# Senpai-sama06/real-time-audio-visual-zooming

Hardware: AMD Instinct MI355X
Metric: beamformed TF-bins/sec (2-ch, 1024-pt STFT) + SIR dB delta vs reference (higher is better)
Workload: dtype f32

## Files before the change

### real-time-audio-visual-zooming_amd/csrc/avz_chain_analysis.hpp

```cpp
#pragma once
#include "avz_chain_common.hpp"
#include "avz_chain_exact.hpp"

namespace avz {
template <int N, int MASK, bool IRM, class TW>
__device__ __forceinline__ void analysis_item(const ChainArgs& A, unsigned char* lds, int c,
                                              int b, int p, int P, int slot, const TW& tw_reg,
                                              const LaneConst<N>& K, int seq) {
  using C = KCfg<N>;
  using G = CGeo<N>;
  constexpr int NT = G::NT, H = G::H, F = G::F, NSLOT = G::NSLOT, BPT = G::BPT, PPL = C::PPL;
  constexpr int FB = (MASK == MASK_IBM) ? NSLOT / 2 : NSLOT;
  static_assert(kChunk % FB == 0, "steps tile the chunk");
  constexpr bool REFBITS = N == 1024 && MASK == MASK_IBM && !IRM && !std::is_same<TW, NoTw>::value;
  constexpr bool SHARE = N == 1024 && MASK != MASK_IPD && !std::is_same<TW, NoTw>::value;
  constexpr bool DLT = MASK == MASK_IBM && !REFBITS;

  const int tid = threadIdx.x;
  const int wave = __builtin_amdgcn_readfirstlane(tid >> 6);
  const int lane = tid & 63;
  const int L = utt_len(A, b);
  const int T = (L + H - 1) / H + 1;
  const int nch = (T + kChunk - 1) / kChunk;
  if (L < N || c >= nch) return;
  if (c == 0 && p == 0 && tid == 0) {
    A.peak_u[b] = 0u;
    if (A.peak && A.normalize != NORM_PEAK) A.peak[b] = 0.0f;
  }
  const int t0 = c * kChunk;
  const int nframes = min(kChunk, T - t0);
  constexpr int SA = kChunk / FB;
  const int s_lo = p * SA / P;
  const int nstep = min((nframes + FB - 1) / FB, (p + 1) * SA / P);
  uint32_t* const pendw = reinterpret_cast<uint32_t*>(lds + G::MISC_OFF + 32 + 12 * (seq & 1));
  if (MASK == MASK_IBM && tid == 0) {
    int z = 0;
    opaque_i(z);
    pendw[0] = (uint32_t)z;
    pendw[1] = (uint32_t)z;
    pendw[2] = (uint32_t)z;
  }

  const typename C::Fft fft = K.fft;
  LaneMap<N> lm;
  {
    int ln = threadIdx.x & 63;
    opaque_i(ln);
    lm.init(ln);
  }
  const float cert_raw = A.ibm_cert * (2.0f / N);
  const WinCoef<N> wc = K.wc;
  const int my_slot = wave * C::FPW + lm.grp;
  cf* my_spec = slot_ptr<N>(lds, my_slot);
  const bool ref = (MASK == MASK_IBM) && (wave * C::FPW >= FB);
  const int my_frame = ref ? my_slot - FB : my_slot;
  const int wave_frame0 = ref ? wave * C::FPW - FB : wave * C::FPW;

  const float* mixb = A.mix + (long long)b * A.mix_stride;
  rsrc_t r_re = make_rsrc(mixb, L), r_im = make_rsrc(mixb + A.ch_stride, L);
  if constexpr (MASK == MASK_IBM) {
    if (ref) {
      r_re = make_rsrc(A.ref_tgt + (long long)b * A.ref_stride, L);
      r_im = make_rsrc(A.ref_int + (long long)b * A.ref_stride, L);
    }
  }
  cf v[PPL];
  auto issue_loads = [&](int step) {
    if constexpr (SHARE) {
      const int sp = (t0 + step * FB + wave_frame0) * H - N / 2 + lm.in0;
      if (t0 + step * FB + wave_frame0 >= 1)
        pair_loads<true>(v, r_re, r_im, sp, lm.grp);
      else
        pair_loads<false>(v, r_re, r_im, sp, lm.grp);
      return;
    }
    const int s0 = (t0 + step * FB + my_frame) * H - N / 2 + lm.in0;
    if (t0 + step * FB + wave_frame0 >= 1) {
// ... 3 lines not shown
      });
    } else {
      static_for<0, PPL>([&](auto r) {
        v[r].x = bload(r_re, s0 + C::IN_STRIDE * r);
        v[r].y = bload(r_im, s0 + C::IN_STRIDE * r);
      });
    }
  };

  constexpr bool IL_LOADS = N == 1024 && !std::is_same<TW, NoTw>::value;
  const rsrc_t r_none = make_rsrc(nullptr, 0);
  rsrc_t rn_re = r_none, rn_im = r_none;
  int sp_next = 0;
  auto load_reg = [&](auto kc) {
    constexpr int k = decltype(kc)::value;
    if constexpr (SHARE) {
      if constexpr (k < 16) {
        const int e = sp_next + 1024 * lm.grp + 32 * k;
        v[k].x = bload_nn(rn_re, e);
        v[k].y = bload_nn(rn_im, e);
      } else if constexpr ((k - 16) % 2 == 0) {
        const int e = sp_next + 512 + 32 * (k - 16) + 32 * lm.grp;
        v[k].x = bload_nn(rn_re, e);
        v[k].y = bload_nn(rn_im, e);
      }
    } else {
      v[k].x = bload_nn(rn_re, sp_next + C::IN_STRIDE * k);
      v[k].y = bload_nn(rn_im, sp_next + C::IN_STRIDE * k);
    }
  };

  Acc32 acc[BPT];
  uint32_t bits[BPT];
  uint32_t dfr[BPT];
  int ipd_clear_n[BPT];
#pragma unroll
  for (int j = 0; j < BPT; ++j) {
    acc[j].zero();
    bits[j] = 0u;
    dfr[j] = 0u;
    ipd_clear_n[j] = 0;
  }
  static_assert(!IRM || MASK == MASK_IBM, "IRM needs the references");
  float* const gain = IRM ? A.pf_gain + ((long long)b * A.nchunk + c) * kChunk * F : nullptr;
  const bool nyq_wave = (wave == G::NWAVE - 1);
  Acc32 an, adc;
  an.zero();
  adc.zero();
  uint32_t nyq_bits = 0u, nyq_dfr = 0u;
  float wone[BPT];
#pragma unroll
  for (int j = 0; j < BPT; ++j) wone[j] = (MASK == MASK_IPD && j == 0 && tid == 0) ? 0.0f : 1.0f;

  AVZ_STAMP_DECL();
  issue_loads(s_lo);
  lds_barrier();
  AVZ_STAMP_INIT();
  for (int step = s_lo; step < nstep; ++step) {
    const int f0 = t0 + step * FB;
    const bool live = f0 + wave_frame0 < T;
#ifdef AVZ_STAMPS
    asm volatile("s_waitcnt vmcnt(0)" ::: "memory");
    AVZ_STAMP(0);
#endif
    if (live) {
      if constexpr (SHARE) pair_finish(v);
      float eg0 = 0.0f, eg1 = eg0;
      if constexpr (REFBITS) {
        if (ref) {
          const float eg = group32_sum(frame_energy(v));
          int e0 = __builtin_amdgcn_readlane(__float_as_int(eg), 0);
          int e1 = __builtin_amdgcn_readlane(__float_as_int(eg), 32);
          const bool o0 = (uint32_t)e0 - A.ibm_en_lo > A.ibm_en_span;
          const bool o1 = (uint32_t)e1 - A.ibm_en_lo > A.ibm_en_span;
          if ((o0 || o1) && A.ibm_cert > 0.0f) {
            uint32_t nz = 0u;
            static_for<0, 32>([&](auto r) { nz |= __float_as_uint(v[r].x) | __float_as_uint(v[r].y); });
            const unsigned long long any = __ballot((nz << 1) != 0u);
            const bool f0 = o0 && (uint32_t)any != 0u, f1 = o1 && (any >> 32) != 0ull;
            if (f0 || f1) {
              const bool mine = lm.grp ? f1 : f0;
              static_for<0, 32>([&](auto r) {
                v[r].x = mine ? 0.0f : v[r].x;
                v[r].y = mine ? 0.0f : v[r].y;
              });
              e0 = f0 ? 0x7f800000 : e0;
              e1 = f1 ? 0x7f800000 : e1;
            }
          }
          eg0 = __int_as_float(e0);
          eg1 = __int_as_float(e1);
        }
      }
      if constexpr (MASK == MASK_IPD) {
        bool same = true;
        static_for<0, PPL>([&](auto r) {
          same &= __float_as_uint(v[r].x) == __float_as_uint(v[r].y);
        });
        const unsigned long long nb = __ballot(!same);
        const bool ident = (C::FPW == 1) ? nb == 0ull : ((nb >> (32 * lm.grp)) & 0xffffffffull) == 0ull;
        if ((lane & (64 / C::FPW - 1)) == 0) lds[G::MISC_OFF + my_slot] = ident ? 1 : 0;
      }
      if constexpr (IL_LOADS) {
        const bool more = step + 1 < nstep;
        rn_re = more ? r_re : r_none;
        rn_im = more ? r_im : r_none;
        sp_next = (t0 + (step + 1) * FB + (SHARE ? wave_frame0 : my_frame)) * H - N / 2 + lm.in0;
      }
      float en = 0.0f;
      if constexpr (!IL_LOADS) {
        window_fft<N>(v, wc, fft, my_spec, lm, NoAfter{}, (DLT && ref) ? &en : nullptr);
      } else if constexpr (REFBITS) {
        uint32_t um = 0u;
        if (step + 1 < nstep) {
          if (ref)
            um = window_fft_reg_ibm_bits(v, wc, fft, my_spec, tw_reg, lm, eg0, eg1, cert_raw, en,
// ... 178 lines not shown
        const bool dc = (j == 0 && tid == 0);
        if (dc) f = 0u;
        ipd_clear_n[j] += dc ? 0 : nvalid - __popc(f);
        while (f) {
          const int i = __builtin_ctz(f);
          f &= f - 1u;
          const cf* Zm = slot_ptr<N>(lds, i);
          cf x0, x1;
          split_pair2(Zm[kb], Zm[kp], x0, x1);
          const float w = ((ident_w >> (8 * i)) & 1ull) ? 0.01f : ipd_weight_exact(x0, x1);
          acc[j].add(x0, x1, w - 1.0f, w);
        }
      }
    }
    if (nyq_wave) {
      bool noise = false, nunc = false;
      if (lane < nvalid) {
        int ln = lane;
        opaque_i(ln);
        const cf* Zm = slot_ptr<N>(lds, ln);
        cf y0, y1, zr{0, 0};
        split_pair2(Zm[N / 2], Zm[N / 2], y0, y1);
        if constexpr (MASK == MASK_IBM) zr = slot_ptr<N>(lds, FB + ln)[N / 2];
        float wn;
        float mn = bin_mask<MASK>(A, b, y0, y1, zr, zr, N / 2, f0 + lane, noise, wn);
        if (MASK == MASK_IPD && ((ident_w >> (8 * lane)) & 1ull)) wn = mn = 0.01f;
        if (MASK == MASK_IBM &&
            ibm_uncertain(zr, zr, reinterpret_cast<const float*>(lds + G::MISC_OFF + 16)[lane])) {
          noise = false;
          wn = mn = 0.0f;
          nunc = true;
          atomicOr(pendw, 1u << (step * FB + lane));
        }
        an.add(y0, y1, wn, mn);
        if constexpr (MASK == MASK_IPD) {
          cf d0, d1;
          const cf z0 = Zm[0];
          split_pair2(z0, z0, d0, d1);
          const float wd = ((ident_w >> (8 * lane)) & 1ull) ? 0.01f : ipd_weight_exact(d0, d1);
          adc.add(d0, d1, wd, wd);
        }
        if constexpr (IRM) gain[(step * FB + lane) * F + N / 2] = irm_gain(zr, zr);
      }
      const unsigned long long bal = __ballot(noise);
      nyq_bits |= ((uint32_t)bal & ((1u << FB) - 1u)) << (step * FB);
      if constexpr (MASK == MASK_IBM)
        nyq_dfr |= ((uint32_t)__ballot(nunc) & ((1u << FB) - 1u)) << (step * FB);
    }
    AVZ_STAMP(12);
    lds_barrier();
    AVZ_STAMP(2);
  }

  if constexpr (MASK == MASK_IBM) {
    const uint32_t pend = pendw[0], full = pendw[1];
    const uint32_t big = REFBITS ? pendw[2] : pend;
    KArgs& Ak = kernarg_chain_args();
    const int gxi = (Ak.max_frames + kChunk - 1) / kChunk;
    const int unit = slot < 0 ? b * gxi + c : gxi * Ak.batch + slot;
    if (nyq_wave && lane == 0) {
      reinterpret_cast<uint4*>(Ak.xpend)[unit] = make_uint4(pend, full, nyq_dfr, big);
      if (pend) *reinterpret_cast<uint32_t*>(lds + G::MISC_OFF + 56) |= 1u << min(seq, 31);
    }
    if (DLT && pend != 0u) {
#pragma unroll
      for (int j = 0; j < BPT; ++j) Ak.xdfr[(long long)unit * F + tid + j * NT] = dfr[j];
    }
  }

  float* Pt = slot < 0 ? A.part + ((long long)b * A.nchunk + c) * 5 * F
                       : A.tpart + (long long)slot * 5 * F;
  uint32_t* MW = A.mwords + ((long long)b * A.nchunk + c) * F;
  const uint32_t rng = (P == 1) ? ~0u : ((1u << (kChunk / P)) - 1u) << (kChunk / P * p);
  auto put_word = [&](int k, uint32_t w) {
    if (slot < 0) {
      MW[k] = w;
    } else {
      atomicAnd(MW + k, ~rng);
      atomicOr(MW + k, w);
    }
  };
  constexpr bool DC_NYQ = MASK == MASK_IPD;
#pragma unroll
  for (int j = 0; j < BPT; ++j) {
    const int kb = tid + j * NT;
    if (DC_NYQ && kb == 0) continue;
    if constexpr (MASK == MASK_IBM) acc[j].cm = (float)__popc(bits[j]);
    if constexpr (MASK == MASK_IPD) acc[j].cm += (float)ipd_clear_n[j];
    Pt[0 * F + kb] = acc[j].c00;
    Pt[1 * F + kb] = acc[j].c11;
    Pt[2 * F + kb] = acc[j].c01r;
    Pt[3 * F + kb] = acc[j].c01i;
    Pt[4 * F + kb] = acc[j].cm;
    if constexpr (MASK == MASK_IBM) put_word(kb, bits[j]);
  }
  if (nyq_wave) {
    for (int o = 1; o < 64; o <<= 1) {
      an.c00 += __shfl_xor(an.c00, o, 64);
      an.c11 += __shfl_xor(an.c11, o, 64);
      an.c01r += __shfl_xor(an.c01r, o, 64);
      an.c01i += __shfl_xor(an.c01i, o, 64);
      an.cm += __shfl_xor(an.cm, o, 64);
      if constexpr (DC_NYQ) {
        adc.c00 += __shfl_xor(adc.c00, o, 64);
        adc.c11 += __shfl_xor(adc.c11, o, 64);
        adc.c01r += __shfl_xor(adc.c01r, o, 64);
        adc.c01i += __shfl_xor(adc.c01i, o, 64);
        adc.cm += __shfl_xor(adc.cm, o, 64);
      }
    }
    if (DC_NYQ && lane == 0) {
      Pt[0 * F] = adc.c00;
      Pt[1 * F] = adc.c11;
      Pt[2 * F] = adc.c01r;
      Pt[3 * F] = adc.c01i;
      Pt[4 * F] = adc.cm;
    }
    if (lane == 0) {
      Pt[0 * F + N / 2] = an.c00;
      Pt[1 * F + N / 2] = an.c11;
      Pt[2 * F + N / 2] = an.c01r;
      Pt[3 * F + N / 2] = an.c01i;
      Pt[4 * F + N / 2] = an.cm;
      if constexpr (MASK == MASK_IBM) put_word(N / 2, nyq_bits);
    }
  }

  if constexpr (MASK == MASK_IBM) {
    const uint32_t big = REFBITS ? pendw[2] : pendw[0];
    if (big != 0u) {
      AVZ_XT_BEGIN(tp);
      __syncthreads();
      if (tid == 0) {
        KArgs& Ak = kernarg_chain_args();
        const int gxi = (Ak.max_frames + kChunk - 1) / kChunk;
        const int unit = slot < 0 ? b * gxi + c : gxi * Ak.batch + slot;
        const XPieces q = x_pieces(pendw[0], big);
        Ak.xst[2 * unit + 1] = 0u;
        __builtin_amdgcn_fence(__ATOMIC_RELEASE, "agent");
        __hip_atomic_store(Ak.xst + 2 * unit, kXOpen | ((uint32_t)q.n << 16), __ATOMIC_RELAXED,
                           __HIP_MEMORY_SCOPE_AGENT);
        __hip_atomic_fetch_or(Ak.xhint + (unit >> 5), 1u << (unit & 31), __ATOMIC_RELAXED,
                              __HIP_MEMORY_SCOPE_AGENT);
#ifdef AVZ_XTRACE
        if (g_stamps) {
          g_stamps[blockIdx.x * 16 + 12] += __builtin_amdgcn_s_memrealtime() - tp;
          g_stamps[blockIdx.x * 16 + 13] += 1 + 256 * q.n;
        }
#endif
      }
    }
  }
}

template <int N, int MASK, bool IRM, bool SPLIT, class TW>
__device__ __forceinline__ void analysis_items(const ChainArgs& A, unsigned char* lds, int gx,
                                               int n_items, const TW& tw_reg,
                                               const LaneConst<N>& K) {
  const int P = SPLIT && A.a_pieces > 1 ? A.a_pieces : 1;
  const int n_whole = P > 1 ? A.a_whole : n_items;
  const int n_end = n_whole + (n_items - n_whole) * P;
  int seq = 0;
  for (int u = blockIdx.x; u < n_end; u += gridDim.x) {
    const bool whole = u < n_whole;
    const int q = u - n_whole, it = whole ? u : n_whole + q / P;
    analysis_item<N, MASK, IRM>(A, lds, it % gx, it / gx, whole ? 0 : q % P, whole ? 1 : P,
                                whole ? -1 : q, tw_reg, K, seq++);
  }
}

template <int N, int MASK, bool IRM, bool SPLIT = false>
__global__ void __launch_bounds__(kCThreads, KCfg<N>::BLOCKS_PER_CU) avz_analysis_kernel(ChainArgs A) {
  using G = CGeo<N>;
  extern __shared__ __align__(16) unsigned char lds[];
  AVZ_XT(0, __builtin_amdgcn_s_memrealtime());
  if (MASK == MASK_IBM && threadIdx.x == 0)
    *reinterpret_cast<uint32_t*>(lds + G::MISC_OFF + 56) = 0u;
  if (A.pstate)
    for (int b = blockIdx.x * kCThreads + threadIdx.x; b < A.batch; b += gridDim.x * kCThreads)
      A.pstate[b] = PieceState{};
  KCfg<N>::Fft::fill_twiddles(reinterpret_cast<cf*>(lds + G::TW_OFF), threadIdx.x, G::NT);
  const int gx = (A.max_frames + kChunk - 1) / kChunk;
  const int n_items = gx * A.batch;
  if constexpr (N == 1024) {
    __syncthreads();
    cf tw_reg[31];
    Fft1024x2 f;
    f.init(threadIdx.x & 63);
    f.load_twiddles(tw_reg, reinterpret_cast<const cf*>(lds + G::TW_OFF));
    if (MASK != MASK_IPD && (threadIdx.x & 32)) {
      static_for<0, 16>([&](auto i) { tw_reg[2 * i] = cf{-tw_reg[2 * i].x, -tw_reg[2 * i].y}; });
    }
    LaneConst<N> K;
    K.init(threadIdx.x);
    if (MASK != MASK_IPD && (threadIdx.x & 32)) {
      K.wc.ac = -K.wc.ac;
      K.wc.as = -K.wc.as;
    }
    analysis_items<N, MASK, IRM, SPLIT>(A, lds, gx, n_items, tw_reg, K);
    if constexpr (MASK == MASK_IBM) ibm_exact_units<N, MASK, IRM, SPLIT, Tw1024>(lds, gx, n_items);
  } else {
    LaneConst<N> K;
    K.init(threadIdx.x);
    analysis_items<N, MASK, IRM, SPLIT>(A, lds, gx, n_items, NoTw{}, K);
    if constexpr (MASK == MASK_IBM) ibm_exact_units<N, MASK, IRM, SPLIT, NoTw>(lds, gx, n_items);
  }
}
}
```

### real-time-audio-visual-zooming_amd/csrc/avz_chain_solve.hpp

```cpp
#pragma once
#include "avz_chain_common.hpp"

namespace avz {
constexpr int kSolveThreads = 256;

template <int N, int V = 8, bool SPLIT = true>
__device__ __forceinline__ void bin_cov_sums(const ChainArgs& A, int b, int k, int nch,
                                             double (&R)[5]) {
  constexpr int F = N / 2 + 1;
  const float* P = A.part + (long long)b * A.nchunk * 5 * F + k;
#pragma unroll
  for (int q = 0; q < 5; ++q) R[q] = 0.0;
  const long long it0 = (long long)b * ((A.max_frames + kChunk - 1) / kChunk);
  const int cw =
      SPLIT && A.a_pieces > 1 ? (int)max(0LL, min((long long)nch, A.a_whole - it0)) : nch;
  for (int cc = 0; cc < cw; ++cc) {
#pragma unroll
    for (int q = 0; q < 5; ++q) R[q] += (double)P[((long long)cc * 5 + q) * F];
  }
  if (SPLIT && cw < nch) {
    const int nv = (nch - cw) * A.a_pieces;
    const rsrc_t rt =
        make_rsrc(A.tpart + (it0 + cw - A.a_whole) * A.a_pieces * 5 * F, (long long)nv * 5 * F);
    for (int v0 = 0; v0 < nv; v0 += V) {
      float p[V][5];
#pragma unroll
      for (int i = 0; i < V; ++i)
#pragma unroll
        for (int q = 0; q < 5; ++q) p[i][q] = bload_nn(rt, ((v0 + i) * 5 + q) * F + k);
#pragma unroll
      for (int i = 0; i < V; ++i)
#pragma unroll
        for (int q = 0; q < 5; ++q) R[q] += (double)p[i][q];
    }
  }
#pragma unroll
  for (int q = 0; q < 4; ++q) R[q] *= 0.25;
}
template <int N, bool SPLIT = true, int VF = 4>
__device__ __forceinline__ void bin_cov_sums_utt(const ChainArgs& A, int b, int k, int nch,
                                                 double (&R)[5]) {
  constexpr int F = N / 2 + 1;
  if (SPLIT && A.a_pieces > 1 &&
      (long long)b * ((A.max_frames + kChunk - 1) / kChunk) + nch > A.a_whole) {
    bin_cov_sums<N, VF>(A, b, k, nch, R);
    return;
  }
  const rsrc_t rp = make_rsrc(A.part + (long long)b * A.nchunk * 5 * F, (long long)nch * 5 * F);
#pragma unroll
  for (int q = 0; q < 5; ++q) R[q] = 0.0;
  for (int c0 = 0; c0 < nch; c0 += 4) {
    float p[4][5];
#pragma unroll
    for (int i = 0; i < 4; ++i)
#pragma unroll
      for (int q = 0; q < 5; ++q) p[i][q] = bload_nn(rp, ((c0 + i) * 5 + q) * F + k);
#pragma unroll
    for (int i = 0; i < 4; ++i)
#pragma unroll
      for (int q = 0; q < 5; ++q) R[q] += (double)p[i][q];
  }
#pragma unroll
  for (int q = 0; q < 4; ++q) R[q] *= 0.25;
}
template <int N>
__device__ __forceinline__ void solve_bin_out(const ChainArgs& A, int b, int k,
                                              const double (&R)[5]) {
  constexpr int F = N / 2 + 1;
  if (A.cov_only) {
#pragma unroll
    for (int q = 0; q < 5; ++q) A.cov_out[((long long)b * F + k) * 5 + q] = R[q];
    return;
  }
  const double* d = A.steer + 4 * k;
  cf al, be;
  float* wdbg = A.w_out ? A.w_out + ((long long)b * F + k) * 4 : nullptr;
  if (A.beamformer == BF_HYBRID_NULL) {
    hybrid_solve_d(R, k, N, A, d[0], d[1], d[2], d[3], al, be, wdbg);
  } else {
    double w[4];
    bool sing = false;
    mvdr_weights_d(R, k, N, A, d[0], d[1], d[2], d[3], w, &sing);
    if (sing && A.singular_fallback == 2) atomicOr(A.flag + b, 1);
    coef_from_w(w[0], w[1], w[2], w[3], al, be, wdbg);
  }
  reinterpret_cast<float4*>(A.coef)[(long long)b * F + k] = make_float4(al.x, al.y, be.x, be.y);
  if (A.cov_out) {
#pragma unroll
    for (int q = 0; q < 5; ++q) A.cov_out[((long long)b * F + k) * 5 + q] = R[q];
  }
}

template <int N, bool SPLIT = false>
__global__ void __launch_bounds__(kSolveThreads) avz_solve_kernel(ChainArgs A) {
  constexpr int H = N / 2, F = N / 2 + 1;
  const long long idx = (long long)blockIdx.x * kSolveThreads + threadIdx.x;
  if (idx >= (long long)(A.batch - A.b_lo) * F) return;
  const int b = A.b_lo + (int)(idx / F), k = (int)(idx % F);
  const int L = utt_len(A, b);
  if (L < N) return;
  const int T = (L + H - 1) / H + 1;
  const int nch = (T + kChunk - 1) / kChunk;
  double R[5];
  bin_cov_sums<N, 8, SPLIT>(A, b, k, nch, R);
  solve_bin_out<N>(A, b, k, R);
}

constexpr int kSolveLanes = 8;
template <int N>
__global__ void __launch_bounds__(kSolveThreads) avz_solve_lanes_kernel(ChainArgs A) {
  constexpr int H = N / 2, F = N / 2 + 1, V = 20;
  const int sub = threadIdx.x % kSolveLanes;
  const long long idx = (long long)blockIdx.x * (kSolveThreads / kSolveLanes) +
// ... 114 lines not shown
```

### real-time-audio-visual-zooming_amd/csrc/avz_chain_utt.hpp

```cpp
#pragma once
#include "avz_chain_common.hpp"
#include "avz_chain_solve.hpp"

namespace avz {
constexpr int kUttThreads = 512;
struct UttGeo {
  static constexpr int N = 1024, H = 512, F = 513, FB = 16;
  static constexpr int SLOT = KCfg<1024>::GROUP_BYTES;
  static constexpr int TW_OFF = FB * SLOT;
  static constexpr int COEF_OFF = TW_OFF + KCfg<1024>::TW_BYTES;
  static constexpr int RED_OFF = COEF_OFF + F * 16;
  static constexpr int LDS_BYTES = RED_OFF + 64;
  static_assert(LDS_BYTES <= 160 * 1024, "one block per CU");
  static_assert(kChunk % FB == 0, "a step stays inside one 32-frame mask chunk");
};
__device__ __forceinline__ cf* utt_frame(unsigned char* lds, int f) {
  return reinterpret_cast<cf*>(lds + f * UttGeo::SLOT);
}

template <int PF, bool SOLVE, bool PIECES>
__global__ void __launch_bounds__(kUttThreads, 2) avz_synthesis_utt_kernel(ChainArgs A) {
  constexpr int N = UttGeo::N, H = UttGeo::H, F = UttGeo::F, FB = UttGeo::FB;
  extern __shared__ __align__(16) unsigned char lds[];
  cf* twid = reinterpret_cast<cf*>(lds + UttGeo::TW_OFF);
  float* red = reinterpret_cast<float*>(lds + UttGeo::RED_OFF);
  Fft1024x2::fill_twiddles(twid, threadIdx.x, kUttThreads);
  const int tid = threadIdx.x;
  const int wave = __builtin_amdgcn_readfirstlane(tid >> 6);
  const int lane = tid & 63;
  Fft1024x2 fft;
  fft.init(lane);
  LaneMap<N> lm;
  lm.init(lane);
  if (lm.grp) {
    static_for<0, 4>([&](auto i) { fft.twa[2 * i] = cf{-fft.twa[2 * i].x, -fft.twa[2 * i].y}; });
  }
  const WinCoef<N> wc0 = [&] {
    WinCoef<N> w;
    w.init(lm);
    if (lm.grp) {
      w.ac = -w.ac;
      w.as = -w.as;
    }
    return w;
  }();
  const int my = 2 * wave + lm.grp;
  cf om[4];
#pragma unroll
  for (int j = 0; j < 4; ++j) {
    double sn, cs;
    sincospi(2.0 * (lane + 64 * j) / N, &sn, &cs);
    om[j] = cf{(float)cs, (float)sn};
  }
  float wh_c[2], wh_s[2];
  const int mh = (lane & 15) + 256 * ((lane >> 4) & 1);
#pragma unroll
  for (int e = 0; e < 2; ++e) {
    double sn, cs;
    sincospi(2.0 * (2 * mh + e) / N, &sn, &cs);
    wh_c[e] = (float)(0.25 * cs);
    wh_s[e] = (float)(0.25 * sn);
  }
  float inv[4];
  __syncthreads();
  AVZ_STAMP_DECL();
  AVZ_STAMP_INIT();

  const int pieces = PIECES && A.s_pieces > 0 ? A.s_pieces : 0;
  const int s_whole = pieces > 0 ? A.s_whole : A.batch;
  const bool ipf = PIECES && pieces > 0 && A.s_ipf;
  const int G = gridDim.x;
  const int n_pu = (A.batch - s_whole) * pieces;
  const int n_units = ipf ? G + s_whole : s_whole + n_pu;
  struct Unit {
    int g, b, s_lo, s_hi, slot;
  };
  auto unit_at = [&](int g) -> Unit {
    for (; g < n_units; g += gridDim.x) {
      const bool is_whole = ipf ? g >= G : g < s_whole;
      if (is_whole) {
        const int gw = ipf ? g - G : g;
        const int Lg = __builtin_amdgcn_readfirstlane(utt_len(A, gw));
        if (Lg >= N) return Unit{g, gw, 0, ((Lg + H - 1) / H + 1 + FB - 1) / FB, -1};
        if (tid == 0 && A.peak) A.peak[gw] = __builtin_nanf("");
        continue;
      }
      const int pc = pieces > 0 ? pieces : 1;
      const int q = ipf ? g : g - s_whole;
      if (q >= n_pu) continue;
      const int bq = s_whole + q / pc, lo = (q % pc) * A.s_steps;
      const int Lq = __builtin_amdgcn_readfirstlane(utt_len(A, bq));
      const int ns = ((Lq + H - 1) / H + 1 + FB - 1) / FB;
      if (Lq >= N && lo < ns) return Unit{g, bq, lo, min(ns, lo + A.s_steps), q};
      if (ipf && Lq < N && lo == 0 && tid == 0 && A.peak) A.peak[bq] = __builtin_nanf("");
    }
    return Unit{n_units, A.batch, 0, 0, -1};
  };
  auto rsrcs = [&](int bb, rsrc_t& a0, rsrc_t& a1) {
    bb = __builtin_amdgcn_readfirstlane(bb);
    const float* mixb = A.mix + (long long)bb * A.mix_stride;
    const int len = __builtin_amdgcn_readfirstlane(utt_len(A, bb));
    a0 = make_rsrc(mixb, len);
    a1 = make_rsrc(mixb + A.ch_stride, len);
  };
  cf v[32];
  auto first_loads = [&](rsrc_t a0, rsrc_t a1, int f0) {
    const int sp = (f0 + 2 * wave) * H - N / 2 + lm.in0;
    if (wave >= 1 || f0 > 0)
      pair_loads<true>(v, a0, a1, sp, lm.grp);
    else
      pair_loads<false>(v, a0, a1, sp, lm.grp);
    (void)my;
  };
  auto solve_coefs = [&](int bb, int TT, auto vf) {
    constexpr int VF = decltype(vf)::value;
    float4* ct = reinterpret_cast<float4*>(lds + UttGeo::COEF_OFF);
    const int nch = (TT + kChunk - 1) / kChunk;
    for (int k = tid; k < F; k += kUttThreads) {
      double R[5], w[4];
      bin_cov_sums_utt<N, PIECES, VF>(A, bb, k, nch, R);
      const double* d = A.steer + 4 * k;
      mvdr_weights_d(R, k, N, A, d[0], d[1], d[2], d[3], w, nullptr);
      cf al, be;
      coef_from_w(w[0], w[1], w[2], w[3], al, be, nullptr);
      ct[k] = make_float4(al.x, al.y, be.x, be.y);
    }
  };
  Unit cu = unit_at(blockIdx.x);
  bool coefs_ready = false;
  if (PIECES && SOLVE && cu.slot >= 0) {
    const int Lp = __builtin_amdgcn_readfirstlane(utt_len(A, cu.b));
    solve_coefs(cu.b, (Lp + H - 1) / H + 1, std::integral_constant<int, 16>{});
    coefs_ready = true;
  }
#pragma unroll
  for (int i = 0; i < 4; ++i) inv[i] = inv_wsum<N>(4 * (tid & 127) + i);
  if (cu.b < A.batch) {
    rsrc_t a0, a1;
    rsrcs(cu.b, a0, a1);
    first_loads(a0, a1, PIECES ? cu.s_lo * FB : 0);
  }
  float* rs_out = nullptr;
  float rs_scale = 0.0f;
  int rs_n4 = 0, rs_done = 0;
  constexpr int RS_U = 4;
  constexpr int RS_UP = 8;
  constexpr int RS_BULK = 32;
  int rs_lazy = -1, rs_lp = 0;
  uint32_t* redu = reinterpret_cast<uint32_t*>(red);
  auto rescale_slice = [&](auto uc, int lo, int hi, auto issue_more) -> bool {
    constexpr int U = decltype(uc)::value;
    const rsrc_t ro = make_rsrc(rs_out, 4LL * rs_n4);
    int tq = tid;
    if constexpr (PIECES) opaque_i(tq);
    float4 x[U];
#pragma unroll
    for (int u = 0; u < U; ++u) {
      const v4i_t d = __builtin_amdgcn_raw_buffer_load_b128(ro, 16 * (lo + u * kUttThreads + tq), 0,
                                                            kSC1);
      x[u] = make_float4(__int_as_float(d.x), __int_as_float(d.y), __int_as_float(d.z),
                         __int_as_float(d.w));
    }
    uint32_t fb = 0;
    if (PIECES && rs_lazy >= 0)
      fb = __hip_atomic_load(&A.pstate[rs_lazy].fin, __ATOMIC_RELAXED, __HIP_MEMORY_SCOPE_AGENT);
    issue_more();
    if (PIECES && rs_lazy >= 0) {
      fb = __builtin_amdgcn_readfirstlane(fb);
      if (fb == 0u || A.dbg_ipf == 2) return false;
      rs_scale = __uint_as_float(fb);
      rs_lazy = -1;
    }
    float4* o4 = reinterpret_cast<float4*>(rs_out);
#pragma unroll
    for (int u = 0; u < U; ++u) {
      const int i = lo + u * kUttThreads + tq;
      if (i < hi) {
        x[u].x *= rs_scale; x[u].y *= rs_scale; x[u].z *= rs_scale; x[u].w *= rs_scale;
        o4[i] = x[u];
      }
    }
    return true;
  };
  auto rescale_rest = [&](auto uc) {
    constexpr int U = decltype(uc)::value;
    for (; rs_done < rs_n4; rs_done += U * kUttThreads)
      rescale_slice(uc, rs_done, min(rs_n4, rs_done + U * kUttThreads), [] {});
    rs_out = nullptr;
  };
  auto rs_resolve = [&]() {
    const uint32_t fb = redu[12];
    const unsigned long long st = *reinterpret_cast<const unsigned long long*>(redu + 10);
    if (fb != 0u) {
// ... 48 lines not shown
    }
    for (int o = 32; o > 0; o >>= 1) mx = fmaxf(mx, __shfl_xor(mx, o, 64));
    __syncthreads();
    if (lane == 0) red[wave] = mx;
    if (t == 0) redu[9] = pku;
    __syncthreads();
    float pk = __uint_as_float(redu[9]);
#pragma unroll
    for (int w = 0; w < kUttThreads / 64; ++w) pk = fmaxf(pk, red[w]);
    const float scale = 1.0f / (pk + A.norm_eps);
    float* ot = outb + t;
    for (int p = 1; p < np; ++p) ot[(long long)(p * sg - 1) * H] = stash[(p - 1) * H] * scale;
    if (t == 0) {
      if (A.peak) A.peak[b] = pk;
      __hip_atomic_store(&A.pstate[b].fin, __float_as_uint(scale), __ATOMIC_RELAXED,
                         __HIP_MEMORY_SCOPE_AGENT);
      asm volatile("s_waitcnt vmcnt(0)" ::: "memory");
      uint32_t hi;
      asm volatile("v_mov_b32 %0, -1" : "=v"(hi));
      const unsigned long long old = atomicOr(&A.pstate[b].st, (unsigned long long)hi << 32);
      *reinterpret_cast<unsigned long long*>(redu + 10) = old;
      if ((uint32_t)old != 0u) __builtin_amdgcn_fence(__ATOMIC_ACQUIRE, "agent");
    }
    __syncthreads();
    const unsigned long long hb = *reinterpret_cast<const unsigned long long*>(redu + 10);
    for (int p = 0; p < np; ++p)
      if ((hb >> p) & 1ull) {
        rs_out = outb;
        rs_scale = scale;
        rs_done = piece_lo4(p, sg);
        rs_n4 = piece_hi4(p, sg, T);
        rescale_rest(std::integral_constant<int, 2 * RS_U>{});
      }
  };
  const int seg = FB * (A.s_steps > 0 ? A.s_steps : 1);
  while (cu.b < A.batch) {
    const int b = cu.b;
    const int L = __builtin_amdgcn_readfirstlane(utt_len(A, b));
    const int T = (L + H - 1) / H + 1;
    rsrc_t r0, r1;
    rsrcs(b, r0, r1);
    int nb = 0, nlen = 0, nf0 = 0;
    {
      const Unit t = unit_at(cu.g + gridDim.x);
      if (t.b < A.batch) {
        nb = __builtin_amdgcn_readfirstlane(t.b);
        nlen = __builtin_amdgcn_readfirstlane(utt_len(A, t.b));
        nf0 = PIECES ? __builtin_amdgcn_readfirstlane(t.s_lo * FB) : 0;
      }
    }
    {
      float4* ct = reinterpret_cast<float4*>(lds + UttGeo::COEF_OFF);
      if (SOLVE) {
        if (!PIECES || !coefs_ready) solve_coefs(b, T, std::integral_constant<int, 4>{});
        coefs_ready = false;
      } else {
        const float4* coef = reinterpret_cast<const float4*>(A.coef) + (long long)b * F;
        int k0 = tid;
        opaque_i(k0);
        for (int k = k0; k < F; k += kUttThreads) ct[k] = coef[k];
      }
    }
    __syncthreads();
    AVZ_STAMP(15);
    uint32_t bits[9];
    float4 carry = make_float4(0.f, 0.f, 0.f, 0.f);
    float peak = 0.0f;
    float* outb = A.out + (long long)b * A.out_stride;
    const int s_hi = cu.s_hi, s_lo = PIECES ? cu.s_lo : 0;
    int step = s_lo;
    for (; step < s_hi; ++step) {
#ifdef AVZ_STAMPS
      asm volatile("s_waitcnt vmcnt(0)" ::: "memory");
      AVZ_STAMP(13);
#endif
      const int f0 = step * FB, c = f0 / kChunk;
      int ln = lane, tq = tid;
      opaque_i(ln);
      opaque_i(tq);
      if ((f0 % kChunk == 0 || (PIECES && step == s_lo)) && PF == PF_IBM_TARGET) {
        const uint32_t* MW = A.mwords + ((long long)b * A.nchunk + c) * F;
#pragma unroll
        for (int q = 0; q < 9; ++q)
          bits[q] = MW[q < 4 ? ln + 64 * q : (q < 8 ? H - ln - 64 * (q - 4) : N / 4)];
      }
      const bool more = step + 1 < s_hi;
      const bool il = more || wave >= 1 || nf0 > 0;
      rsrc_t q0, q1;
      {
        const int qb = __builtin_amdgcn_readfirstlane(more ? b : nb);
        const int ql = __builtin_amdgcn_readfirstlane(more ? L : nlen);
        const float* qm = A.mix + (long long)qb * A.mix_stride;
        q0 = make_rsrc(qm, ql);
        q1 = make_rsrc(qm + A.ch_stride, ql);
      }
      const int sn = ((more ? f0 + FB : nf0) + 2 * wave) * H - N / 2 + lm.in0;
      auto load_k = [&](auto kc) {
        constexpr int k = decltype(kc)::value;
        if constexpr (k < 16) {
          const int e = sn + 1024 * lm.grp + 32 * k;
          v[k].x = bload_nn(q0, e);
          v[k].y = bload_nn(q1, e);
        } else if constexpr ((k - 16) % 2 == 0) {
          const int e = sn + 512 + 32 * (k - 16) + 32 * lm.grp;
          v[k].x = bload_nn(q0, e);
          v[k].y = bload_nn(q1, e);
        }
      };
      auto next_loads = [&]() {
        if (il)
          static_for<0, 32>(load_k);
        else
          first_loads(q0, q1, 0);
      };
      pair_finish(v);
      window_fft<N>(v, wc0, fft, utt_frame(lds, my), lm);
      AVZ_STAMP(4);
      __builtin_amdgcn_wave_barrier();
      const float* irm = (PF == PF_IRM) ? A.pf_gain + ((long long)b * A.nchunk + c) * kChunk * F
                                        : nullptr;
      auto gain = [&](uint32_t bb, int i, int t, int k) -> float {
        if (t >= T) return 0.0f;
        if constexpr (PF == PF_IBM_TARGET) {
          return ((bb >> i) & 1u) ? 0.0f : 1.0f;
        } else if constexpr (PF == PF_IRM) {
          return irm[i * F + k];
        } else if constexpr (PF == PF_EXT_FLOOR || PF == PF_EXT_MUL) {
// ... 478 lines not shown
```

### real-time-audio-visual-zooming_amd/csrc/avz_common.hpp

```cpp
#pragma once
#include <hip/hip_runtime.h>
#include <stdint.h>

#include <atomic>

#include "avz_fft.hpp"
#include "avz_internal.h"

namespace avz {

typedef __amdgpu_buffer_rsrc_t rsrc_t;

__device__ __forceinline__ rsrc_t make_rsrc(const float* p, long long n_floats) {
  long long bytes = (p == nullptr || n_floats <= 0) ? 0 : n_floats * 4;
  if (bytes > 0x7fffffffLL) bytes = 0x7fffffffLL;
  return __builtin_amdgcn_make_buffer_rsrc((void*)p, (short)0, (int)bytes, 0x00020000);
}

__device__ __forceinline__ float bload(rsrc_t r, int elem) {
  const unsigned off = (elem < 0) ? 0xfffffffcu : (unsigned)elem * 4u;
  return __uint_as_float(__builtin_amdgcn_raw_buffer_load_b32(r, (int)off, 0, 0));
}

#ifdef AVZ_STAMPS
#ifndef AVZ_STAMP_WAVE
#define AVZ_STAMP_WAVE 0
#endif
static __device__ unsigned long long* g_stamps;
#define AVZ_STAMP_DECL() unsigned long long stamp_prev = 0
#define AVZ_STAMP_INIT() stamp_prev = __builtin_amdgcn_s_memrealtime()
#define AVZ_STAMP(i)                                                        \
  do {                                                                      \
    if (threadIdx.x == 64 * AVZ_STAMP_WAVE && g_stamps) {                   \
      const unsigned long long now_ = __builtin_amdgcn_s_memrealtime();     \
      atomicAdd(g_stamps + (blockIdx.y * gridDim.x + blockIdx.x) * 16 + (i), now_ - stamp_prev); \
      stamp_prev = now_;                                                    \
    }                                                                       \
  } while (0)
#else
#define AVZ_STAMP_DECL() (void)0
#define AVZ_STAMP_INIT() (void)0
#define AVZ_STAMP(i) (void)0
#endif
#ifdef AVZ_XTRACE
#ifndef AVZ_STAMPS
static __device__ unsigned long long* g_stamps;
#endif
#define AVZ_XT(i, v)                                                                    \
  do {                                                                                  \
    if (threadIdx.x == 0 && g_stamps)                                                   \
      g_stamps[(blockIdx.y * gridDim.x + blockIdx.x) * 16 + (i)] = (unsigned long long)(v); \
  } while (0)
#define AVZ_XT_BEGIN(t) const unsigned long long t = __builtin_amdgcn_s_memrealtime()
#define AVZ_XT_END(i, t)                                                                \
  do {                                                                                  \
    if (threadIdx.x == 0 && g_stamps)                                                   \
      g_stamps[blockIdx.x * 16 + (i)] += __builtin_amdgcn_s_memrealtime() - (t);        \
  } while (0)
#define AVZ_XT_LAP_BEGIN(t) unsigned long long t = __builtin_amdgcn_s_memrealtime()
#define AVZ_XT_LAP(i, t)                                                                \
  do {                                                                                  \
    if (threadIdx.x == 0 && g_stamps) {                                                 \
      const unsigned long long now_ = __builtin_amdgcn_s_memrealtime();                 \
      g_stamps[blockIdx.x * 16 + (i)] += now_ - t;                                      \
      t = now_;                                                                         \
    }                                                                                   \
  } while (0)
#else
#define AVZ_XT(i, v) (void)0
#define AVZ_XT_LAP_BEGIN(t) (void)0
#define AVZ_XT_LAP(i, t) (void)0
#define AVZ_XT_BEGIN(t) (void)0
#define AVZ_XT_END(i, t) (void)0
#endif

__device__ __forceinline__ float bload_nn(rsrc_t r, int elem) {
  return __uint_as_float(__builtin_amdgcn_raw_buffer_load_b32(r, elem * 4, 0, 0));
}

__device__ __forceinline__ void opaque(float& x) { asm volatile("" : "+v"(x)); }
__device__ __forceinline__ void opaque_i(int& x) { asm volatile("" : "+v"(x)); }

__device__ __forceinline__ void lds_barrier() {
  __builtin_amdgcn_fence(__ATOMIC_RELEASE, "workgroup", "local");
  __builtin_amdgcn_s_barrier();
  __builtin_amdgcn_fence(__ATOMIC_ACQUIRE, "workgroup", "local");
}

template <int N>
struct KCfg;
template <>
struct KCfg<1024> {
  using Fft = Fft1024x2;
  static constexpr int PPL = Fft::PPL;
  static constexpr int FPW = 2;
// ... 309 lines not shown
```

Baseline: 79.77 billion.

## Issue first frame and covariance-part loads before twiddle setup in utterance kernel

In the non-pieces utterance kernel, the first unit lookup, the first frame loads and the first group of covariance partial loads are now issued before twiddle fill and per-lane constant setup. This hides global memory latency behind prologue work and drops a block-wide barrier. The per-bin solve is split into an issue phase and a finish phase, and a single thread also handles the Nyquist bin so the bin loop is no longer strided. Edge-timestamp instrumentation macros are added as well; they compile to nothing by default. The cost is extra registers held live across the prologue, which could reduce occupancy.

```diff
diff --git a/real-time-audio-visual-zooming_amd/csrc/avz_chain_analysis.hpp b/real-time-audio-visual-zooming_amd/csrc/avz_chain_analysis.hpp
--- a/real-time-audio-visual-zooming_amd/csrc/avz_chain_analysis.hpp
+++ b/real-time-audio-visual-zooming_amd/csrc/avz_chain_analysis.hpp
@@ -23,6 +23,8 @@
   const int T = (L + H - 1) / H + 1;
   const int nch = (T + kChunk - 1) / kChunk;
   if (L < N || c >= nch) return;
+  AVZ_STAMP_DECL();
+  AVZ_STAMP_EDGE_OPEN(seq == 0 ? 1 : 2);
   if (c == 0 && p == 0 && tid == 0) {
     A.peak_u[b] = 0u;
     if (A.peak && A.normalize != NORM_PEAK) A.peak[b] = 0.0f;
@@ -132,7 +134,6 @@
 #pragma unroll
   for (int j = 0; j < BPT; ++j) wone[j] = (MASK == MASK_IPD && j == 0 && tid == 0) ? 0.0f : 1.0f;
 
-  AVZ_STAMP_DECL();
   issue_loads(s_lo);
   lds_barrier();
   AVZ_STAMP_INIT();
@@ -142,6 +143,10 @@
 #ifdef AVZ_STAMPS
     asm volatile("s_waitcnt vmcnt(0)" ::: "memory");
     AVZ_STAMP(0);
+    if (step == s_lo) {
+      AVZ_STAMP_EDGE_CLOSE(seq == 0 ? 1 : 2);
+      if (seq == 0) AVZ_STAMP_EDGE_CLOSE(0);
+    }
 #endif
     if (live) {
       if constexpr (SHARE) pair_finish(v);
@@ -426,6 +431,7 @@
     AVZ_STAMP(2);
   }
 
+  AVZ_STAMP_EDGE_OPEN(3);
   if constexpr (MASK == MASK_IBM) {
     const uint32_t pend = pendw[0], full = pendw[1];
     const uint32_t big = REFBITS ? pendw[2] : pend;
@@ -525,6 +531,7 @@
       }
     }
   }
+  AVZ_STAMP_EDGE_CLOSE(3);
 }
 
 template <int N, int MASK, bool IRM, bool SPLIT, class TW>
@@ -548,6 +555,7 @@
   using G = CGeo<N>;
   extern __shared__ __align__(16) unsigned char lds[];
   AVZ_XT(0, __builtin_amdgcn_s_memrealtime());
+  AVZ_STAMP_EDGE_OPEN(0);
   if (MASK == MASK_IBM && threadIdx.x == 0)
     *reinterpret_cast<uint32_t*>(lds + G::MISC_OFF + 56) = 0u;
   if (A.pstate)
diff --git a/real-time-audio-visual-zooming_amd/csrc/avz_chain_solve.hpp b/real-time-audio-visual-zooming_amd/csrc/avz_chain_solve.hpp
--- a/real-time-audio-visual-zooming_amd/csrc/avz_chain_solve.hpp
+++ b/real-time-audio-visual-zooming_amd/csrc/avz_chain_solve.hpp
@@ -37,6 +37,20 @@
 #pragma unroll
   for (int q = 0; q < 4; ++q) R[q] *= 0.25;
 }
+template <int N>
+__device__ __forceinline__ void bin_part_loads4(rsrc_t rp, int c0, int k, float (&p)[4][5]) {
+  constexpr int F = N / 2 + 1;
+#pragma unroll
+  for (int i = 0; i < 4; ++i)
+#pragma unroll
+    for (int q = 0; q < 5; ++q) p[i][q] = bload_nn(rp, ((c0 + i) * 5 + q) * F + k);
+}
+__device__ __forceinline__ void bin_part_add4(const float (&p)[4][5], double (&R)[5]) {
+#pragma unroll
+  for (int i = 0; i < 4; ++i)
+#pragma unroll
+    for (int q = 0; q < 5; ++q) R[q] += (double)p[i][q];
+}
 template <int N, bool SPLIT = true, int VF = 4>
 __device__ __forceinline__ void bin_cov_sums_utt(const ChainArgs& A, int b, int k, int nch,
                                                  double (&R)[5]) {
@@ -51,14 +65,8 @@
   for (int q = 0; q < 5; ++q) R[q] = 0.0;
   for (int c0 = 0; c0 < nch; c0 += 4) {
     float p[4][5];
-#pragma unroll
-    for (int i = 0; i < 4; ++i)
-#pragma unroll
-      for (int q = 0; q < 5; ++q) p[i][q] = bload_nn(rp, ((c0 + i) * 5 + q) * F + k);
-#pragma unroll
-    for (int i = 0; i < 4; ++i)
-#pragma unroll
-      for (int q = 0; q < 5; ++q) R[q] += (double)p[i][q];
+    bin_part_loads4<N>(rp, c0, k, p);
+    bin_part_add4(p, R);
   }
 #pragma unroll
   for (int q = 0; q < 4; ++q) R[q] *= 0.25;
diff --git a/real-time-audio-visual-zooming_amd/csrc/avz_chain_utt.hpp b/real-time-audio-visual-zooming_amd/csrc/avz_chain_utt.hpp
--- a/real-time-audio-visual-zooming_amd/csrc/avz_chain_utt.hpp
+++ b/real-time-audio-visual-zooming_amd/csrc/avz_chain_utt.hpp
@@ -4,6 +4,9 @@
 
 namespace avz {
 constexpr int kUttThreads = 512;
+#ifndef AVZ_UTT_EARLY
+#define AVZ_UTT_EARLY 1
+#endif
 struct UttGeo {
   static constexpr int N = 1024, H = 512, F = 513, FB = 16;
   static constexpr int SLOT = KCfg<1024>::GROUP_BYTES;
@@ -24,14 +27,137 @@
   extern __shared__ __align__(16) unsigned char lds[];
   cf* twid = reinterpret_cast<cf*>(lds + UttGeo::TW_OFF);
   float* red = reinterpret_cast<float*>(lds + UttGeo::RED_OFF);
-  Fft1024x2::fill_twiddles(twid, threadIdx.x, kUttThreads);
+  AVZ_STAMP_DECL();
+  AVZ_STAMP_EDGE_INIT();
   const int tid = threadIdx.x;
   const int wave = __builtin_amdgcn_readfirstlane(tid >> 6);
   const int lane = tid & 63;
+  LaneMap<N> lm;
+  lm.init(lane);
+  const int my = 2 * wave + lm.grp;
+
+  const int pieces = PIECES && A.s_pieces > 0 ? A.s_pieces : 0;
+  const int s_whole = pieces > 0 ? A.s_whole : A.batch;
+  const bool ipf = PIECES && pieces > 0 && A.s_ipf;
+  const int G = gridDim.x;
+  const int n_pu = (A.batch - s_whole) * pieces;
+  const int n_units = ipf ? G + s_whole : s_whole + n_pu;
+  struct Unit {
+    int g, b, s_lo, s_hi, slot;
+  };
+  auto unit_at = [&](int g) -> Unit {
+    for (; g < n_units; g += gridDim.x) {
+      const bool is_whole = ipf ? g >= G : g < s_whole;
+      if (is_whole) {
+        const int gw = ipf ? g - G : g;
+        const int Lg = __builtin_amdgcn_readfirstlane(utt_len(A, gw));
+        if (Lg >= N) return Unit{g, gw, 0, ((Lg + H - 1) / H + 1 + FB - 1) / FB, -1};
+        if (tid == 0 && A.peak) A.peak[gw] = __builtin_nanf("");
+        continue;
+      }
+      const int pc = pieces > 0 ? pieces : 1;
+      const int q = ipf ? g : g - s_whole;
+      if (q >= n_pu) continue;
+      const int bq = s_whole + q / pc, lo = (q % pc) * A.s_steps;
+      const int Lq = __builtin_amdgcn_readfirstlane(utt_len(A, bq));
+      const int ns = ((Lq + H - 1) / H + 1 + FB - 1) / FB;
+      if (Lq >= N && lo < ns) return Unit{g, bq, lo, min(ns, lo + A.s_steps), q};
+      if (ipf && Lq < N && lo == 0 && tid == 0 && A.peak) A.peak[bq] = __builtin_nanf("");
+    }
+    return Unit{n_units, A.batch, 0, 0, -1};
+  };
+  auto rsrcs = [&](int bb, rsrc_t& a0, rsrc_t& a1) {
+    bb = __builtin_amdgcn_readfirstlane(bb);
+    const float* mixb = A.mix + (long long)bb * A.mix_stride;
+    const int len = __builtin_amdgcn_readfirstlane(utt_len(A, bb));
+    a0 = make_rsrc(mixb, len);
+    a1 = make_rsrc(mixb + A.ch_stride, len);
+  };
+  cf v[32];
+  auto first_loads = [&](rsrc_t a0, rsrc_t a1, int f0) {
+    const int sp = (f0 + 2 * wave) * H - N / 2 + lm.in0;
+    if (wave >= 1 || f0 > 0)
+      pair_loads<true>(v, a0, a1, sp, lm.grp);
+    else
+      pair_loads<false>(v, a0, a1, sp, lm.grp);
+    (void)my;
+  };
+  auto solve_bin = [&](const double (&R)[5], int k) {
+    float4* ct = reinterpret_cast<float4*>(lds + UttGeo::COEF_OFF);
+    double w[4];
+    const double* d = A.steer + 4 * k;
+    mvdr_weights_d(R, k, N, A, d[0], d[1], d[2], d[3], w, nullptr);
+    cf al, be;
+    coef_from_w(w[0], w[1], w[2], w[3], al, be, nullptr);
+    ct[k] = make_float4(al.x, al.y, be.x, be.y);
+  };
+  auto solve_coefs = [&](int bb, int TT, auto vf) {
+    constexpr int VF = decltype(vf)::value;
+    const int nch = (TT + kChunk - 1) / kChunk;
+    for (int k = tid; k < F; k += kUttThreads) {
+      double R[5];
+      bin_cov_sums_utt<N, PIECES, VF>(A, bb, k, nch, R);
+      solve_bin(R, k);
+    }
+  };
+  auto part_rsrc = [&](int bb, int nch) {
+    return make_rsrc(A.part + (long long)bb * A.nchunk * 5 * F, (long long)nch * 5 * F);
+  };
+  auto solve_issue = [&](int bb, int nch, float (&p)[4][5], float (&p2)[4][5]) {
+    const rsrc_t rp = part_rsrc(bb, nch);
+    bin_part_loads4<N>(rp, 0, tid, p);
+    if (tid == 0) bin_part_loads4<N>(rp, 0, N / 2, p2);
+  };
+  auto solve_finish = [&](int bb, int nch, float (&p)[4][5], float (&p2)[4][5]) {
+    const rsrc_t rp = part_rsrc(bb, nch);
+    double R[5], R2[5];
+#pragma unroll
+    for (int q = 0; q < 5; ++q) R[q] = R2[q] = 0.0;
+    bin_part_add4(p, R);
+    if (tid == 0) bin_part_add4(p2, R2);
+    for (int c0 = 4; c0 < nch; c0 += 4) {
+      bin_part_loads4<N>(rp, c0, tid, p);
+      if (tid == 0) bin_part_loads4<N>(rp, c0, N / 2, p2);
+      bin_part_add4(p, R);
+      if (tid == 0) bin_part_add4(p2, R2);
+    }
+    int k = tid;
+#pragma unroll 1
+    for (int j = 0; j < 2; ++j) {
+#pragma unroll
+      for (int q = 0; q < 4; ++q) R[q] *= 0.25;
+      solve_bin(R, k);
+      if (tid != 0) break;
+#pragma unroll
+      for (int q = 0; q < 5; ++q) R[q] = R2[q];
+      k = N / 2;
+    }
+  };
+  constexpr bool EARLY = !PIECES && AVZ_UTT_EARLY;
+  Unit cu = Unit{0, A.batch, 0, 0, -1};
+  float pe[4][5], pe2[4][5];
+#pragma unroll
+  for (int i = 0; i < 4; ++i)
+#pragma unroll
+    for (int q = 0; q < 5; ++q) pe[i][q] = pe2[i][q] = 0.0f;
+  bool pe_issued = false;
+  if constexpr (EARLY) {
+    cu = unit_at(blockIdx.x);
+    if (cu.b < A.batch) {
+      rsrc_t a0, a1;
+      rsrcs(cu.b, a0, a1);
+      first_loads(a0, a1, 0);
+      if constexpr (SOLVE) {
+        const int Le = __builtin_amdgcn_readfirstlane(utt_len(A, cu.b));
+        solve_issue(cu.b, ((Le + H - 1) / H + 1 + kChunk - 1) / kChunk, pe, pe2);
+        pe_issued = true;
+      }
+    }
+  }
+  AVZ_STAMP_EDGE(5);
+  Fft1024x2::fill_twiddles(twid, tid, kUttThreads);
   Fft1024x2 fft;
   fft.init(lane);
-  LaneMap<N> lm;
-  lm.init(lane);
   if (lm.grp) {
     static_for<0, 4>([&](auto i) { fft.twa[2 * i] = cf{-fft.twa[2 * i].x, -fft.twa[2 * i].y}; });
   }
@@ -44,7 +170,6 @@
     }
     return w;
   }();
-  const int my = 2 * wave + lm.grp;
   cf om[4];
 #pragma unroll
   for (int j = 0; j < 4; ++j) {
@@ -62,83 +187,30 @@
     wh_s[e] = (float)(0.25 * sn);
   }
   float inv[4];
-  __syncthreads();
-  AVZ_STAMP_DECL();
-  AVZ_STAMP_INIT();
-
-  const int pieces = PIECES && A.s_pieces > 0 ? A.s_pieces : 0;
-  const int s_whole = pieces > 0 ? A.s_whole : A.batch;
-  const bool ipf = PIECES && pieces > 0 && A.s_ipf;
-  const int G = gridDim.x;
-  const int n_pu = (A.batch - s_whole) * pieces;
-  const int n_units = ipf ? G + s_whole : s_whole + n_pu;
-  struct Unit {
-    int g, b, s_lo, s_hi, slot;
-  };
-  auto unit_at = [&](int g) -> Unit {
-    for (; g < n_units; g += gridDim.x) {
-      const bool is_whole = ipf ? g >= G : g < s_whole;
-      if (is_whole) {
-        const int gw = ipf ? g - G : g;
-        const int Lg = __builtin_amdgcn_readfirstlane(utt_len(A, gw));
-        if (Lg >= N) return Unit{g, gw, 0, ((Lg + H - 1) / H + 1 + FB - 1) / FB, -1};
-        if (tid == 0 && A.peak) A.peak[gw] = __builtin_nanf("");
-        continue;
-      }
-      const int pc = pieces > 0 ? pieces : 1;
-      const int q = ipf ? g : g - s_whole;
-      if (q >= n_pu) continue;
-      const int bq = s_whole + q / pc, lo = (q % pc) * A.s_steps;
-      const int Lq = __builtin_amdgcn_readfirstlane(utt_len(A, bq));
-      const int ns = ((Lq + H - 1) / H + 1 + FB - 1) / FB;
-      if (Lq >= N && lo < ns) return Unit{g, bq, lo, min(ns, lo + A.s_steps), q};
-      if (ipf && Lq < N && lo == 0 && tid == 0 && A.peak) A.peak[bq] = __builtin_nanf("");
-    }
-    return Unit{n_units, A.batch, 0, 0, -1};
-  };
-  auto rsrcs = [&](int bb, rsrc_t& a0, rsrc_t& a1) {
-    bb = __builtin_amdgcn_readfirstlane(bb);
-    const float* mixb = A.mix + (long long)bb * A.mix_stride;
-    const int len = __builtin_amdgcn_readfirstlane(utt_len(A, bb));
-    a0 = make_rsrc(mixb, len);
-    a1 = make_rsrc(mixb + A.ch_stride, len);
-  };
-  cf v[32];
-  auto first_loads = [&](rsrc_t a0, rsrc_t a1, int f0) {
-    const int sp = (f0 + 2 * wave) * H - N / 2 + lm.in0;
-    if (wave >= 1 || f0 > 0)
-      pair_loads<true>(v, a0, a1, sp, lm.grp);
-    else
-      pair_loads<false>(v, a0, a1, sp, lm.grp);
-    (void)my;
-  };
-  auto solve_coefs = [&](int bb, int TT, auto vf) {
-    constexpr int VF = decltype(vf)::value;
-    float4* ct = reinterpret_cast<float4*>(lds + UttGeo::COEF_OFF);
-    const int nch = (TT + kChunk - 1) / kChunk;
-    for (int k = tid; k < F; k += kUttThreads) {
-      double R[5], w[4];
-      bin_cov_sums_utt<N, PIECES, VF>(A, bb, k, nch, R);
-      const double* d = A.steer + 4 * k;
-      mvdr_weights_d(R, k, N, A, d[0], d[1], d[2], d[3], w, nullptr);
-      cf al, be;
-      coef_from_w(w[0], w[1], w[2], w[3], al, be, nullptr);
-      ct[k] = make_float4(al.x, al.y, be.x, be.y);
-    }
-  };
-  Unit cu = unit_at(blockIdx.x);
   bool coefs_ready = false;
-  if (PIECES && SOLVE && cu.slot >= 0) {
-    const int Lp = __builtin_amdgcn_readfirstlane(utt_len(A, cu.b));
-    solve_coefs(cu.b, (Lp + H - 1) / H + 1, std::integral_constant<int, 16>{});
-    coefs_ready = true;
-  }
-#pragma unroll
-  for (int i = 0; i < 4; ++i) inv[i] = inv_wsum<N>(4 * (tid & 127) + i);
-  if (cu.b < A.batch) {
-    rsrc_t a0, a1;
-    rsrcs(cu.b, a0, a1);
-    first_loads(a0, a1, PIECES ? cu.s_lo * FB : 0);
+  if constexpr (EARLY) {
+#pragma unroll
+    for (int i = 0; i < 4; ++i) inv[i] = inv_wsum<N>(4 * (tid & 127) + i);
+    AVZ_STAMP_INIT();
+    AVZ_STAMP_EDGE(4);
+  } else {
+    __syncthreads();
+    AVZ_STAMP_INIT();
+    AVZ_STAMP_EDGE(4);
+    cu = unit_at(blockIdx.x);
+    if (SOLVE && cu.slot >= 0) {
+      const int Lp = __builtin_amdgcn_readfirstlane(utt_len(A, cu.b));
+      solve_coefs(cu.b, (Lp + H - 1) / H + 1, std::integral_constant<int, 16>{});
+      coefs_ready = true;
+    }
+#pragma unroll
+    for (int i = 0; i < 4; ++i) inv[i] = inv_wsum<N>(4 * (tid & 127) + i);
+    if (cu.b < A.batch) {
+      rsrc_t a0, a1;
+      rsrcs(cu.b, a0, a1);
+      first_loads(a0, a1, cu.s_lo * FB);
+    }
+    AVZ_STAMP_EDGE(5);
   }
   float* rs_out = nullptr;
   float rs_scale = 0.0f;
@@ -293,8 +365,20 @@
     {
       float4* ct = reinterpret_cast<float4*>(lds + UttGeo::COEF_OFF);
       if (SOLVE) {
-        if (!PIECES || !coefs_ready) solve_coefs(b, T, std::integral_constant<int, 4>{});
-        coefs_ready = false;
+        if constexpr (PIECES) {
+          if (!coefs_ready) solve_coefs(b, T, std::integral_constant<int, 4>{});
+          coefs_ready = false;
+        } else {
+          const int nch = (T + kChunk - 1) / kChunk;
+          if (!pe_issued) solve_issue(b, nch, pe, pe2);
+          pe_issued = false;
+          solve_finish(b, nch, pe, pe2);
+#pragma unroll
+          for (int i = 0; i < 4; ++i)
+#pragma unroll
+            for (int q = 0; q < 5; ++q) pe[i][q] = pe2[i][q] = 0.0f;
+        }
+        AVZ_STAMP_EDGE(6);
       } else {
         const float4* coef = reinterpret_cast<const float4*>(A.coef) + (long long)b * F;
         int k0 = tid;
@@ -304,6 +388,7 @@
     }
     __syncthreads();
     AVZ_STAMP(15);
+    AVZ_STAMP_EDGE(8);
     uint32_t bits[9];
     float4 carry = make_float4(0.f, 0.f, 0.f, 0.f);
     float peak = 0.0f;
@@ -314,6 +399,10 @@
 #ifdef AVZ_STAMPS
       asm volatile("s_waitcnt vmcnt(0)" ::: "memory");
       AVZ_STAMP(13);
+      if (step == s_lo)
+        AVZ_STAMP_EDGE(9);
+      else
+        AVZ_STAMP_EDGE(10);
 #endif
       const int f0 = step * FB, c = f0 / kChunk;
       int ln = lane, tq = tid;
diff --git a/real-time-audio-visual-zooming_amd/csrc/avz_common.hpp b/real-time-audio-visual-zooming_amd/csrc/avz_common.hpp
--- a/real-time-audio-visual-zooming_amd/csrc/avz_common.hpp
+++ b/real-time-audio-visual-zooming_amd/csrc/avz_common.hpp
@@ -28,8 +28,8 @@
 #endif
 static __device__ unsigned long long* g_stamps;
 #define AVZ_STAMP_DECL() unsigned long long stamp_prev = 0
-#define AVZ_STAMP_INIT() stamp_prev = __builtin_amdgcn_s_memrealtime()
-#define AVZ_STAMP(i)                                                        \
+#define AVZ_STAMP_NOW() stamp_prev = __builtin_amdgcn_s_memrealtime()
+#define AVZ_STAMP_DO(i)                                                    \
   do {                                                                      \
     if (threadIdx.x == 64 * AVZ_STAMP_WAVE && g_stamps) {                   \
       const unsigned long long now_ = __builtin_amdgcn_s_memrealtime();     \
@@ -37,10 +37,35 @@
       stamp_prev = now_;                                                    \
     }                                                                       \
   } while (0)
+#ifdef AVZ_STAMPS_EDGE
+#define AVZ_STAMP_INIT() (void)0
+#define AVZ_STAMP(i) (void)0
+#define AVZ_STAMP_EDGE_INIT() AVZ_STAMP_NOW()
+#define AVZ_STAMP_EDGE(i) AVZ_STAMP_DO(i)
+#define AVZ_STAMP_EDGE_MARK(i, op)                                          \
+  do {                                                                      \
+    if (threadIdx.x == 64 * AVZ_STAMP_WAVE && g_stamps)                     \
+      g_stamps[(blockIdx.y * gridDim.x + blockIdx.x) * 16 + (i)] op         \
+          __builtin_amdgcn_s_memrealtime();                                 \
+  } while (0)
+#define AVZ_STAMP_EDGE_OPEN(i) AVZ_STAMP_EDGE_MARK(i, -=)
+#define AVZ_STAMP_EDGE_CLOSE(i) AVZ_STAMP_EDGE_MARK(i, +=)
+#else
+#define AVZ_STAMP_INIT() AVZ_STAMP_NOW()
+#define AVZ_STAMP(i) AVZ_STAMP_DO(i)
+#define AVZ_STAMP_EDGE_INIT() (void)0
+#define AVZ_STAMP_EDGE(i) (void)0
+#define AVZ_STAMP_EDGE_OPEN(i) (void)0
+#define AVZ_STAMP_EDGE_CLOSE(i) (void)0
+#endif
 #else
 #define AVZ_STAMP_DECL() (void)0
 #define AVZ_STAMP_INIT() (void)0
 #define AVZ_STAMP(i) (void)0
+#define AVZ_STAMP_EDGE_INIT() (void)0
+#define AVZ_STAMP_EDGE(i) (void)0
+#define AVZ_STAMP_EDGE_OPEN(i) (void)0
+#define AVZ_STAMP_EDGE_CLOSE(i) (void)0
 #endif
 #ifdef AVZ_XTRACE
 #ifndef AVZ_STAMPS
```

After: 78.53 billion. 1.6% lower.
